# williamyang1991/VToonify

Hardware: AMD Instinct MI355X
Metric: frames/sec at 1024x1024 VToonify-D inference (higher is better)
Workload: dtype bf16

## Files before the change

include/vtoonify_amd.h:

```cpp
#ifndef VTOONIFY_AMD_H
#define VTOONIFY_AMD_H

#include <stdint.h>

#ifdef __cplusplus
extern "C" {
#endif

#define VT_ABI_VERSION 5

enum { VT_F32 = 0, VT_BF16 = 1, VT_F16 = 2,
       VT_F32X3 = 3,
       VT_F64 = 4 };
enum { VT_OK = 0, VT_ERR_ARG = 1, VT_ERR_UNSUPPORTED = 2, VT_ERR_LAUNCH = 3 };

enum { VT_ACT_NONE = 0, VT_ACT_LRELU = 1, VT_ACT_RELU_TANH = 2, VT_ACT_SIGMOID = 3, VT_ACT_TANH = 4  };
enum { VT_OUT_NHWC = 0, VT_OUT_NCHW = 1 };

typedef void* vt_stream;

int vt_abi_version(void);
const char* vt_last_error(void);
const char* vt_build_target(void);

// ... 161 lines not shown

int vt_nchw_to_nhwc(void* out, int ld_out, const void* in, int n, int c, int hw,
                    int in_dtype, int out_dtype, vt_stream stream);
int vt_nhwc_to_nchw(void* out, const void* in, int ld_in, int n, int c, int hw,
                    int in_dtype, int out_dtype, vt_stream stream);

int vt_mfma_selftest(float* c, const void* a, const void* b, int dtype, vt_stream stream);

#ifdef __cplusplus
}
#endif

#include "vtoonify_amd_prepass.h"
#include "vtoonify_amd_frames.h"
#include "vtoonify_amd_fusion.h"
#endif
```

vtoonify_amd/_lib.py:

```python
from __future__ import annotations

import ctypes as C
import os

HERE = os.path.dirname(os.path.abspath(__file__))
DEFAULT_LIB = os.path.join(HERE, "lib", "libvtoonify_amd.so")

ABI_VERSION = 5
VT_F32, VT_BF16, VT_F16 = 0, 1, 2
VT_F64 = 4
VT_F32X3 = 3
ACT_NONE, ACT_LRELU, ACT_RELU_TANH, ACT_SIGMOID, ACT_TANH = 0, 1, 2, 3, 4
OUT_NHWC, OUT_NCHW = 0, 1


class VtError(RuntimeError):
    pass


class ConvDesc(C.Structure):
    _fields_ = [
        ("src0", C.c_void_p), ("src1", C.c_void_p),
        ("c0", C.c_int32), ("c1", C.c_int32), ("ld0", C.c_int32), ("ld1", C.c_int32),
        ("n", C.c_int32), ("h", C.c_int32), ("w", C.c_int32),
# ... 116 lines not shown
}
PREPASS_SYMBOLS = tuple(_PREPASS_SIGS)

_FRAMES_SIGS = {
    "vt_frame_scale_crop": (C.c_int, [C.c_void_p, C.c_void_p] + [C.c_int] * 6 + [C.c_void_p, C.c_void_p, C.c_int, C.c_int,
                                                                               C.c_void_p]),
}
FRAMES_SYMBOLS = tuple(_FRAMES_SIGS)

_FUSION_SIGS = {
    "vt_conv2d_gate": (C.c_int, [C.POINTER(ConvDesc), C.c_void_p, C.c_int32, C.c_void_p]),
    "vt_conv2d_hdr": (C.c_int, [C.POINTER(ConvDesc), C.c_void_p, C.c_int32, C.c_int32, C.c_void_p]),
}
FUSION_SYMBOLS = tuple(_FUSION_SIGS)

_lib = None
_lib_path = None


def _bind(path: str):
    import torch
    lib = C.CDLL(path)
    for name, (res, args) in {**_SIGS, **_PREPASS_SIGS, **_FRAMES_SIGS, **_FUSION_SIGS}.items():
        fn = getattr(lib, name)
        fn.restype = res
        fn.argtypes = args
    if lib.vt_abi_version() != ABI_VERSION:
        raise VtError(f"{path}: ABI version {lib.vt_abi_version()} != {ABI_VERSION}")
    return lib


def use_library(path: str):
    global _lib, _lib_path
    _lib = _bind(path)
    _lib_path = path
    return _lib


# ... 35 lines not shown
```

vtoonify_amd/csrc/conv_igemm.hip:

```cpp
#include <stdlib.h>
#include <type_traits>
#include <utility>

#include "vt_common.hpp"

namespace {

#ifdef VT_EMU
typedef emu_f32x4 f32x4;
#else
typedef float f32x4 __attribute__((ext_vector_type(4)));
typedef __bf16 bf16x8_t __attribute__((ext_vector_type(8)));
typedef _Float16 f16x8_t __attribute__((ext_vector_type(8)));
#endif

static inline int slab_ld(int cout_total) { return (cout_total + 31) / 32 * 32; }
constexpr int64_t VT_TICKET_BYTES = 16384;

struct ConvArgs {
    const void* src0;
    const void* src1;
    const void* wgt;
    const float* bias;
    const float* slope_vec;
// ... 1337 lines not shown
        vt_lds_barrier();
        if (a_age < 99) ++a_age;
        bbuf = (bbuf + 1 == NSTB) ? 0 : bbuf + 1;
        nbbuf = (nbbuf + 1 == NSTB) ? 0 : nbbuf + 1;
        if (++tap == 9) {
            tap = 0;
            ++chunk;
            if (ABUF == 2) abuf ^= 1;
            a_age = 99;
        }
    }
    __syncthreads();
    conv_epilogue<T, BM, BN, WM, WN>(p, acc, smem, PatchRows<TW>{img, y0, x0, p.Ho, p.Wo}, n0, split, tile_n * p.tiles_m + tile_m);
}

template <typename T>
__global__ void __launch_bounds__(256, 2)
conv3x3_c32_kernel(const ConvArgs p, const GldsArgs g) {
    static_assert(is_h16<T>::value, "16-bit operands only (64-byte pixel rows)");
    constexpr int TH = 16, TW = 16, BM = 256, BN = 32, WM = 4, WN = 1;
    constexpr int TM = 4, TN = 2;
    constexpr int PH = TH + 2, PW = TW + 2, PROWS = PH * PW;
    constexpr int PA = ((PROWS + 15) / 16 + 3) / 4;
    constexpr int A_BYTES = PA * 4 * 1024;
    constexpr int NBUF = 3;
    __shared__ __attribute__((aligned(1024))) unsigned char smem[NBUF * A_BYTES];

    const int tid = threadIdx.x;
    const int lane = tid & 63;
    const int wave = vt_uniform(tid >> 6) & 3;
    const int wm = wave;
    const int q = lane >> 4, l15 = lane & 15;
    auto swz = [](int pr) -> int { return ((pr >> 2) & 1) << 1; };

// ... 36 lines not shown
        for (int i = 0; i < 4; ++i) bvr[b][i] = 0.0f;
    u128 rwf = u128{0u, 0u, 0u, 0u};
    if (rgbf) {
        const bool okw = (l15 & 3) < 3;
        const u128 wv = ld128((const T*)p.rgb_w + (okw ? (l15 & 3) * 32 + q * 8 : 0));
        rwf.x = okw ? wv.x : 0u, rwf.y = okw ? wv.y : 0u, rwf.z = okw ? wv.z : 0u, rwf.w = okw ? wv.w : 0u;
    }
    if (p.bias) {
#pragma unroll
        for (int b = 0; b < TN; ++b)
#pragma unroll
            for (int i = 0; i < 4; ++i) bvr[b][i] = p.bias[cg + frag_channel<true>(b, q) + i];
    }
    float rb0 = 0.0f, rb1 = 0.0f, rb2 = 0.0f;
    if (rgbf && p.rgb_bias) rb0 = p.rgb_bias[0], rb1 = p.rgb_bias[1], rb2 = p.rgb_bias[2];

    int tile = blockIdx.x;
    if (tile >= ntiles) return;
    issue(tile, 0);
    if (tile + (int)gridDim.x < ntiles) issue(tile + (int)gridDim.x, 1);
    int buf = 0;
    for (; tile < ntiles; tile += gridDim.x) {
        const int next2 = tile + 2 * (int)gridDim.x;
        if (next2 < ntiles) {
            issue(next2, buf == 0 ? 2 : buf - 1);
            vt_glds_wait_n<2 * PA>();
        } else if (tile + (int)gridDim.x < ntiles) {
            vt_glds_wait_n<PA>();
        } else {
            vt_glds_wait_n<0>();
// ... 1 lines not shown
        vt_lds_barrier();
        const int img = tile / (tiles_x * tiles_y);
        const int trem = tile - img * (tiles_x * tiles_y);
        const int y0 = (trem / tiles_x) * TH, x0 = (trem % tiles_x) * TW;
        const PatchRows<TW> rowmap{img, y0, x0, p.Ho, p.Wo};
        const int HoWo = p.Ho * p.Wo;
        static_assert(TM == 4, "one tile row per lane group");
        float rsd[3] = {0.0f, 0.0f, 0.0f};
        const int m_rgb = rowmap(wm * (TM * 16) + q * 16 + l15);
        int64_t o_rgb = 0;
        {
            const int mm = m_rgb < 0 ? 0 : m_rgb;
            const int im = mm / HoWo;
            o_rgb = (int64_t)im * 3 * HoWo + (mm - im * HoWo);
        }
        if (rgbf && p.rgb_resid) {
#pragma unroll
            for (int j = 0; j < 3; ++j) rsd[j] = p.rgb_resid[o_rgb + (int64_t)j * HoWo];
        }
        f32x4 acc[TM][TN];
#pragma unroll
        for (int a = 0; a < TM; ++a)
#pragma unroll
            for (int b = 0; b < TN; ++b) acc[a][b] = f32x4{0.f, 0.f, 0.f, 0.f};
        const unsigned char* sa = smem + buf * A_BYTES;
#pragma unroll
        for (int t = 0; t < 9; ++t) {
            const int ky = t / 3, kx = t - ky * 3;
            u128 fa[TM];
#pragma unroll
            for (int a = 0; a < TM; ++a) {
// ... 21 lines not shown
                        if (p.act == VT_ACT_LRELU) v = (v > 0.0f) ? v : v * p.slope;
                        f[4 * b + i] = v * ga;
                    }
                }
                const u128 fpk = pack16<T>(f);
                if (rgbf) {
                    const bool mine = (l15 >> 2) == a;
                    u128 wa;
                    wa.x = mine ? rwf.x : 0u, wa.y = mine ? rwf.y : 0u, wa.z = mine ? rwf.z : 0u, wa.w = mine ? rwf.w : 0u;
                    Mma<T>::run(racc, wa, fpk);
                }
                if (m >= 0 && !p.rgb_only) st128((T*)p.out + (int64_t)m * p.ld_out + cg + q * 8, fpk);
            }
            if (rgbf) {
                const float rr[3] = {racc[0], racc[1], racc[2]};
                if (m_rgb >= 0) {
                    p.rgb_out[o_rgb] = rr[0] + rb0 + rsd[0];
                    p.rgb_out[o_rgb + HoWo] = rr[1] + rb1 + rsd[1];
                    p.rgb_out[o_rgb + 2 * (int64_t)HoWo] = rr[2] + rb2 + rsd[2];
                }
            }
        }
        vt_lds_barrier();
        buf = buf + 1 == NBUF ? 0 : buf + 1;
    }
}

template <int... I, typename F>
__device__ __forceinline__ void vt_static_for_impl(std::integer_sequence<int, I...>, F&& f) {
    (f(std::integral_constant<int, I>{}), ...);
// ... 712 lines not shown
    if (args.phase != 2) {
        if (args.splitk == 1 && conv_lean<T>(args)) {
            auto k = conv_patchc_kernel<T, TH, BN, WM, WN, 1, DIL>;
            VT_LAUNCH(k, dim3((unsigned)blocks), dim3(WM * WN * 64), stream, args, g);
        } else {
            auto k = conv_patchc_kernel<T, TH, BN, WM, WN, 0, DIL>;
            VT_LAUNCH(k, dim3((unsigned)blocks), dim3(WM * WN * 64), stream, args, g);
        }
    }
    int rc = vt_check_launch("vt_conv2d(patch, chunk barriers)");
    if (rc != VT_OK || args.splitk == 1 || args.tickets || args.phase == 1) return rc;
    return launch_reduce<T>(args, stream);
}

template <typename T, int TH, int BN>
int launch_patchw(const ConvArgs& a, const GldsArgs& g, vt_stream stream) {
    ConvArgs args = a;
    args.slab_perm = ((BN / 16) % 2 == 0) ? 1 : 0;
    args.tiles_n = 1;
    args.tiles_m = a.N * vt_cdiv(a.Ho, TH) * vt_cdiv(a.Wo, 16);
    args.kps = 1;
    args.splitk = 1;
    split_mode(args);
    int wgs = patchw_wgs();
    if (wgs > args.tiles_m) wgs = args.tiles_m;
    if (wgs >= 8) wgs &= ~7;
    auto k = conv_patchw_kernel<T, TH, BN>;
    VT_LAUNCH(k, dim3((unsigned)wgs), dim3(512), stream, args, g);
    return vt_check_launch("vt_conv2d(patch, weights resident)");
}

template <typename T>
int launch_c32(const ConvArgs& a, const GldsArgs& g, vt_stream stream) {
    ConvArgs args = a;
    args.slab_perm = 0;
    args.splitk = 1;
    args.tiles_n = 1;
    args.tiles_m = a.N * vt_cdiv(a.Ho, 16) * vt_cdiv(a.Wo, 16);
    const int groups = a.cout / 32;
    const int per_group = 512 / groups > 0 ? 512 / groups : 1;
    int blocks = args.tiles_m < per_group ? args.tiles_m : per_group;
    if (const char* e = getenv("VT_C32_BLOCKS")) {
        const int v = atoi(e);
        if (v > 0 && v < blocks) blocks = v;
    }
    auto k = conv3x3_c32_kernel<T>;
    VT_LAUNCH(k, dim3((unsigned)blocks, (unsigned)groups), dim3(256), stream, args, g);
    return vt_check_launch("vt_conv2d(c32)");
}

template <typename T>
int dispatch(const ConvArgs& a0, int hint, int64_t ws_floats, vt_stream stream) {
    ConvArgs a = a0;
    a.force_generic = hint >= 1000000000 || !axes_equal(a);
    const TilePlan t = choose_plan<T>(a, hint % 1000000000, ws_floats);
    a.splitk = t.splitk;
    a.ldp = slab_ld(a.coutT);
    if (a.rgb_w && (t.bn < a.coutT || t.splitk > 1)) {
        vt_set_error("vt_conv2d: fused ToRGB needs all %d output channels in one tile (plan %dx%d, split %d)",
                     a.coutT, t.bm, t.bn, t.splitk);
        return VT_ERR_UNSUPPORTED;
    }
    if (a.in_absdiff && t.kind != 6) {
        vt_set_error("vt_conv2d: in_absdiff needs the thin-output kernel (plan kind %d)", t.kind);
        return VT_ERR_UNSUPPORTED;
    }
    if (a.rgb_only && t.kind != 3) {
        vt_set_error("vt_conv2d: rgb_only needs the persistent 32 -> 32 kernel (plan kind %d)", t.kind);
        return VT_ERR_UNSUPPORTED;
    }
    if (t.kind == 5) {
        const int chunks = a.cin / (8 * (16 / (int)sizeof(T)));
// ... 54 lines not shown
    }
    if (t.kind == 4) {
        FullkArgs fg;
        if (!fullk_eligible<T>(a, a.wstream, fg)) {
            vt_set_error("vt_conv2d: whole-K kernel requested for an ineligible convolution");
            return VT_ERR_UNSUPPORTED;
        }
        return launch_fullk<T>(a, fg, stream);
    }
    if (t.kind == 3) {
        GldsArgs g;
        if (!c32_eligible<T>(a, g)) {
            vt_set_error("vt_conv2d: c32 kernel requested for an ineligible convolution");
            return VT_ERR_UNSUPPORTED;
        }
        if constexpr (is_h16<T>::value) return launch_c32<T>(a, g, stream);
    }
    if (t.kind == 1 && a.transposed) {
        GldsArgs g;
        if (!up_eligible<T>(a, g)) {
            vt_set_error("vt_conv2d: transposed patch plan requested for an ineligible convolution");
            return VT_ERR_UNSUPPORTED;
        }
        return launch_patchp<T, 16, 64, 4, 2, 8, 1>(a, g, stream);
    }
    if (t.kind == 1) {
        GldsArgs g;
        if (!patch_eligible<T>(a, g)) {
            vt_set_error("vt_conv2d: patch kernel requested for an ineligible convolution");
            return VT_ERR_UNSUPPORTED;
        }
// ... 2 lines not shown
#define VT_PATCH(TH_, BN_, WM_, WN_, DIL_, NSTB_, ABUF_, COND_) \
    if (t.bm == TH_ * 16 && t.bn == BN_ && a.dil == DIL_ && (COND_))  \
        return launch_patch<T, TH_, BN_, WM_, WN_, DIL_, NSTB_, ABUF_>(a, g, stream);
        {
            const char* e = getenv("VT_PATCH_PIPE");
            const bool pipe = !(e && e[0] == '0') && !a.x3;
            if constexpr (is_h16<T>::value) {
                const bool lean = a.coutT == 64 && a.phases == 1 && a.out_layout == VT_OUT_NHWC && !a.out_f32 && a.vec_store &&
                                  a.ld_out % 8 == 0 && !a.resid && !a.slope_vec && !a.alpha_dev && !a.post_relu && !a.stats_part &&
                                  (a.act == VT_ACT_NONE || a.act == VT_ACT_LRELU) &&
                                  (int64_t)a.N * a.Ho * a.Wo * a.ld_out * 2 < (((int64_t)1 << 31) - 4096) &&
                                  (int64_t)a.N * a.Ho * a.Wo * 12 < (((int64_t)1 << 31) - 4096);
                if (pipe && !(e && e[0] == '1') && a.dil == 1 && t.bm == 256 && t.bn == 64 && units == 1 && lean && !a.src1 &&
                    a.splitk <= 1 &&
                    (int64_t)(batch_exact() ? 1 : a.N) * vt_cdiv(a.Ho, 16) * vt_cdiv(a.Wo, 16) >= 2 * patchw_wgs())
                    return launch_patchw<T, 16, 64>(a, g, stream);
            }
            if constexpr (is_h16<T>::value) {
                if (pipe && !(e && e[0] == '1') && a.dil == 1 && t.bm == 256 && (t.bn == 128 || t.bn == 64) && a.splitk <= 1 &&
                    conv_lean<T>(a) && vt_cdiv(a.coutT, t.bn) * t.bn * 8 <= PQ_TAB_BYTES &&
                    (int64_t)a.N * vt_cdiv(a.Ho, 16) * vt_cdiv(a.Wo, 16) * vt_cdiv(a.coutT, t.bn) > patchw_wgs()) {
                    if (t.bn == 128) return launch_patchq<T, 16, 128, 4, 2, 4>(a, g, stream);
                    return launch_patchq<T, 16, 64, 4, 2, 4>(a, g, stream);
                }
            }
            if (pipe && a.dil == 1 && t.bm == 256 && t.bn == 128) return launch_patchp<T, 16, 128, 4, 2>(a, g, stream);
            if (pipe && a.dil == 1 && t.bm == 256 && t.bn == 64) return launch_patchp<T, 16, 64, 4, 2, 4>(a, g, stream);
            if constexpr (is_h16<T>::value) {
                if (pipe && !(e && e[0] == '1') && a.dil == 1 && t.bm == 256 && t.bn == 32) return launch_patchc<T>(a, g, stream);
                if (pipe && !(e && e[0] == '1') && a.dil == 2 && t.bm == 256 && t.bn == 32 && !a.stats_part)
                    return launch_patchc<T, 2>(a, g, stream);
// ... 204 lines not shown
        vt_set_error("vt_conv2d_hdr: needs a 3x3, pad 1 conv of one source with cout <= 3");
        return VT_ERR_UNSUPPORTED;
    }
    if (hdr_c < 0 || hdr_pad <= 0 || hdr_c > hdr_pad || hdr_pad % kstep != 0) {
        vt_set_error("vt_conv2d_hdr: needs 0 <= hdr_c <= hdr_pad, hdr_pad a positive multiple of the K step (%d channels)", kstep);
        return VT_ERR_UNSUPPORTED;
    }
    a.hdr = hdr_planes;
    a.hdr_c = hdr_c;
    a.hdr_pad = hdr_pad;
    a.cin = d->c0 + hdr_pad;
    a.K = a.taps * a.cin;
    return fusion_form_run(d, a, "vt_conv2d_hdr", stream);
}

extern "C" int vt_conv2d_tile(const vt_conv_desc* d) {
    ConvArgs a;
    if (fill_args(d, a) != VT_OK) return -1;
    a.force_generic = d->tile_hint >= 1000000000 || !axes_equal(a);
    const int64_t wsf = (d->splitk_ws && d->splitk_ws_bytes > VT_TICKET_BYTES) ? (d->splitk_ws_bytes - VT_TICKET_BYTES) / 4 : 0;
    const TilePlan t = plan_of(d, a, wsf);
    int kind = t.kind;
    if (kind == 0) {
        GldsArgs g;
        const bool glds = d->dtype == VT_F16    ? glds_eligible<f16_t>(a, g)
                          : d->dtype == VT_BF16 ? glds_eligible<bf16_t>(a, g)
                                                : glds_eligible<float>(a, g);
        kind = glds ? 2 : 0;
    }
    int bm = t.bm, bn = t.bn;
// ... 95 lines not shown
```

vtoonify_amd/csrc/conv_patch_resident.hpp:

```cpp
#pragma once

template <typename T, int TH, int BN>
__global__ void __launch_bounds__(512)
conv_patchw_kernel(const ConvArgs p, const GldsArgs g) {
    constexpr int TW = 16;
    constexpr int GW = 4;
    constexpr int BM = TH * TW;
    constexpr int ESZ = (int)sizeof(T);
    constexpr int TM = BM / GW / 16, TN = BN / 16;
    constexpr bool PERM = (TN % 2 == 0);
    constexpr int PH = TH + 2, PW = TW + 2, PROWS = PH * PW;
    constexpr int NPIECE = (PROWS + 7) / 8;
    constexpr int PA = (NPIECE + GW - 1) / GW;
    constexpr int WPIECE = (BN + 7) / 8;
    constexpr int LB = (WPIECE + 7) / 8;
    constexpr int A_BYTES = NPIECE * 1024, W_TAP = WPIECE * 1024, W_BYTES = 9 * W_TAP;
    constexpr int A_OFF = W_BYTES, TAB_OFF = W_BYTES + 2 * A_BYTES;
    static_assert(sizeof(T) == 2, "bf16 (the lean epilogue packs 8 channels into a 16-byte store)");
    static_assert(BM % (GW * 16) == 0 && BN % 16 == 0, "wave tiling");
    static_assert(TM * GW == TH, "one 16-pixel tile row per MFMA row block");
    static_assert(TAB_OFF + 4 * BN * 4 <= 160 * 1024, "LDS budget");
    static_assert(TM == 4 && TN == 4, "the epilogue below: 4 tile rows per wave (one per lane group), 2 x 32 channels");
    static_assert(9 * LB + PA < 64, "vmcnt is 6 bits");

// ... 58 lines not shown
            if (piece < NPIECE) vt_glds16(r0, smem + aoff + piece * 1024, vo, 0u);
        }
    };
    if (ng > 0) issue_patch(tile_of(0));
    const bool rgbf = p.rgb_w != nullptr;
    if (tid < BN) {
        float* tab = reinterpret_cast<float*>(smem + TAB_OFF);
        tab[tid] = p.bias ? p.bias[tid] : 0.0f;
#pragma unroll
        for (int j = 0; j < 3; ++j) tab[(1 + j) * BN + tid] = rgbf ? to_f32(((const T*)p.rgb_w)[j * p.coutT + tid]) : 0.0f;
    }
    float rb[3] = {0.0f, 0.0f, 0.0f};
    if (rgbf && p.rgb_bias) rb[0] = p.rgb_bias[0], rb[1] = p.rgb_bias[1], rb[2] = p.rgb_bias[2];
    const int HoWo = p.Ho * p.Wo;
    const BufRaw rout = vt_make_raw(p.out, (uint32_t)((int64_t)p.M * p.ld_out * ESZ));
    const BufRaw rskip = vt_make_raw(p.rgb_resid, (uint32_t)((int64_t)p.N * 3 * HoWo * 4));
    const BufRaw rimg = vt_make_raw(p.rgb_out, (uint32_t)((int64_t)p.N * 3 * HoWo * 4));

    const int q = lane >> 4, l15 = lane & 15, l7 = lane & 7;
    uint32_t aswz[8][2];
#pragma unroll
    for (int cm = 0; cm < 8; ++cm)
#pragma unroll
        for (int sub = 0; sub < 2; ++sub)
            aswz[cm][sub] = (uint32_t)(aoff + (wm * TM * PW + l15) * 128 + (((sub * 4 + q) ^ ((wm * TM * PW + l15 + cm) & 7)) << 4));
    uint32_t bfix[2];
#pragma unroll
    for (int sub = 0; sub < 2; ++sub) bfix[sub] = (uint32_t)(l15 * 128 + (((sub * 4 + q) ^ l7) << 4));

    u128 fa[2][TM], fb[2][TN];
    auto read_frags = [&](auto tapc, auto subc, u128 (&xa)[TM], u128 (&xb)[TN]) {
        constexpr int TAP = decltype(tapc)::value, SUB = decltype(subc)::value;
        constexpr int ky = TAP / 3, kx = TAP % 3;
        auto ra = [&](int a) {
// ... 37 lines not shown
        });
        vt_sched_fence();
        vt_lds_barrier();
        if (j + 1 < ng) issue_patch(tile_of(j + 1));
        {
            const int tm = tile_of(j);
            const int im = tm / per_img, tr = tm - im * per_img;
            const PatchRows<TW> rowmap{im, (tr / tiles_x) * TH, (tr % tiles_x) * TW, p.Ho, p.Wo};
            const int m_rgb = rowmap(wm * (TM * 16) + q * 16 + l15);
            uint32_t o_rgb = GLDS_OOB;
            if (m_rgb >= 0) {
                const int ii = m_rgb / HoWo;
                o_rgb = (uint32_t)(ii * 3 * HoWo + (m_rgb - ii * HoWo)) * 4u;
            }
            u128 rsd[3];
            if (rgbf) {
#pragma unroll
                for (int jc = 0; jc < 3; ++jc) vt_bload_hidden<1>(rsd[jc], rskip, m_rgb >= 0 ? o_rgb + (uint32_t)(jc * HoWo) * 4u : GLDS_OOB);
            }
            const float ga = p.gain_alpha;
            const float* tab = reinterpret_cast<const float*>(smem + TAB_OFF);
            f32x4 racc = f32x4{0.f, 0.f, 0.f, 0.f};
            static_assert(TM <= 4 && sizeof(T) == 2, "ToRGB accumulator rows");
#pragma unroll
            for (int hp = 0; hp < 2; ++hp) {
                const int c0 = hp * 32 + q * 8;
                float bv[8];
                unpack16<float>(ld128(tab + c0), bv), unpack16<float>(ld128(tab + c0 + 4), bv + 4);
                u128 wfrag = u128{0u, 0u, 0u, 0u};
                if (rgbf) {
                    const int pl = (l15 & 3) < 3 ? (l15 & 3) : 0;
// ... 17 lines not shown
                    if (rgbf) {
                        const bool mine = (l15 >> 2) == a;
                        u128 wa;
                        wa.x = mine ? wfrag.x : 0u, wa.y = mine ? wfrag.y : 0u, wa.z = mine ? wfrag.z : 0u, wa.w = mine ? wfrag.w : 0u;
                        Mma<T>::run(racc, wa, fpk);
                    }
                    vt_bstore_hidden<4>(rout, m >= 0 ? (uint32_t)(m * p.ld_out + c0) * (uint32_t)ESZ : GLDS_OOB, fpk);
                }
            }
            if (rgbf) {
                const float rr[3] = {racc[0], racc[1], racc[2]};
                vt_vmcnt_fence<2 * TM>();
#pragma unroll
                for (int jc = 0; jc < 3; ++jc) {
                    u128 o;
                    o.x = vt_f2u((rr[jc] + rb[jc]) + vt_u2f(vt_settled(rsd[jc]).x)), o.y = o.z = o.w = 0u;
                    vt_bstore_hidden<1>(rimg, m_rgb >= 0 ? o_rgb + (uint32_t)(jc * HoWo) * 4u : GLDS_OOB, o);
                }
            } else {
                vt_vmcnt_fence<2 * TM>();
            }
        }
        vt_lds_barrier();
    }
    for (int k = grp + 2 * ng; k < nmine + 1; ++k) vt_lds_barrier();
}
```

vtoonify_amd/csrc/vt_common.hpp:

```cpp
#pragma once

#ifndef VT_EMU
#include <hip/hip_runtime.h>
#endif
#include <stdint.h>
#include <stdio.h>
#include <string.h>

#include "../../include/vtoonify_amd.h"

void vt_set_error(const char* fmt, ...);
int vt_check_launch(const char* what);

#define VT_REQUIRE(cond, ...)            \
    do {                                 \
        if (!(cond)) {                   \
            vt_set_error(__VA_ARGS__);   \
            return VT_ERR_ARG;           \
        }                                \
    } while (0)

#ifdef VT_EMU
#define VT_LAUNCH(kern, grid, block, stream, ...) \
    emu::launch((grid), (block), [=]() { kern(__VA_ARGS__); })
// ... 442 lines not shown
    else asm volatile("s_nop 4\n\t" OP_ " %0, %1, %2, 0 offen" ::"v"(X_), "v"(voff), "s"(r.v) : "memory");
    if constexpr (DW == 4) {
        const vt_u32x4 x = __builtin_bit_cast(vt_u32x4, v);
        VT_BST("buffer_store_dwordx4", x)
    } else if constexpr (DW == 2) {
        typedef uint32_t vt_u32x2 __attribute__((ext_vector_type(2)));
        const vt_u32x2 x = {v.x, v.y};
        VT_BST("buffer_store_dwordx2", x)
    } else {
        const uint32_t x = v.x;
        VT_BST("buffer_store_dword", x)
    }
#undef VT_BST
}
#endif

__device__ __forceinline__ float wave_sum(float v) {
#pragma unroll
    for (int off = 32; off > 0; off >>= 1) v += __shfl_xor(v, off, 64);
    return v;
}

static inline int vt_cdiv(int64_t a, int64_t b) { return (int)((a + b - 1) / b); }
__device__ __forceinline__ int vt_cdiv_dev(int a, int b) { return (a + b - 1) / b; }

#ifdef VT_EMU
static inline void vt_wave_sync() {
    const int dummy = 0;
    (void)emu::exchange(&dummy, (int)sizeof(dummy));
}
// ... 17 lines not shown
```

vtoonify_amd/engine.py:

```python
from __future__ import annotations

import ctypes as C
import math
import os
from typing import Dict, List, Optional, Tuple

import torch

from . import _lib
from . import kernels as K
from ._lib import ACT_LRELU, ACT_NONE, ACT_RELU_TANH, OUT_NCHW, OUT_NHWC

SQRT2 = math.sqrt(2.0)
N_LATENT = 18
_DIL = {1: 4, 2: 4, 3: 2, 4: 2, 5: 1, 6: 1}
SKIP_HDR = 64


def _pad8(c: int) -> int:
    return (c + 7) // 8 * 8


class _Plan:
    def __init__(self):
# ... 2 lines not shown
        self.enc_ops: List[Tuple] = []
        self.gen_ops: List[Tuple] = []
        self.keep: list = []
        self.masks: List[torch.Tensor] = []
        self.graphs: dict = {}
        self.convs: list = []


class VToonifyEngine:
    supports_borrow = True

    def __init__(self, state_dict: Dict[str, torch.Tensor], backbone: str = "dualstylegan",
                 in_size: int = 256, dtype: torch.dtype = torch.bfloat16,
                 device: Optional[torch.device] = None, cache_styles: bool = False,
                 tile_hints: Optional[Dict[str, int]] = None, style_gate: bool = False, x3: bool = False,
                 fuse_rgb128: bool = True, fused_gate=True):
        assert backbone in ("dualstylegan", "toonify")
        assert dtype in (torch.bfloat16, torch.float16, torch.float32)
        self.backbone = backbone
        self.dual = backbone == "dualstylegan"
        self.in_size = in_size
        self.dtype = dtype
        self.dt = K.dt_code(dtype)
        self.x3 = bool(x3) and dtype == torch.float32
        self.dt_conv = K.VT_F32X3 if self.x3 else self.dt
        self.h16 = dtype in (torch.bfloat16, torch.float16)
        self.precision = ({torch.bfloat16: "bf16", torch.float16: "fp16"}[dtype] if self.h16 else
                          ("fp32x3" if self.x3 else "fp32_exact"))
        self.esz = 2 if self.h16 else 4
        any_t = next(iter(state_dict.values()))
        self.device = torch.device(device) if device is not None else any_t.device
        if self.device.type == "cuda" and self.device.index is None:
            self.device = torch.device("cuda", torch.cuda.current_device())
        self.lib = _lib.lib()
        if self.device.type != "cuda" and not _lib.is_emulation():
            raise _lib.VtError("VToonifyEngine needs a GPU device (no CPU path)")
        self.cache_styles = cache_styles
        self.fuse_rgb128 = bool(fuse_rgb128)
        self.fused_gate = fused_gate if fused_gate == "all" else bool(fused_gate)
        self.style_gate = bool(style_gate)
        self.graph_first = os.environ.get("VT_GRAPH_FIRST", "1") != "0"
        self.use_upblur = True
        self.tile_hints: Dict[str, int] = dict(tile_hints or {})
        if not self.tile_hints and os.environ.get("VT_TILE_HINTS"):
            import json
            with open(os.environ["VT_TILE_HINTS"]) as f:
                self.tile_hints = {k: int(v) for k, v in json.load(f).items()}
        self.sd = {k: v.detach().to(self.device, torch.float32).contiguous() for k, v in state_dict.items()}
        self.g = "generator.generator." if self.dual else "generator."
        self.n_down = 0
        while f"encoder.{self.n_down}.0.weight" in self.sd:
            self.n_down += 1
        self.n_fuse = sum(1 for lvl in range(5) if 2 ** (5 + lvl) <= in_size)
        import collections
# ... 103 lines not shown
            info["join"] = True
        if entry is not None:
            info["form"] = entry[2]
            info["bytes"] += entry[3]
        plan.convs.append((d, info, ops, len(ops)))
        ops.append((self.lib.vt_conv2d, (C.byref(d),), info) if entry is None else (entry[0], (C.byref(d),) + tuple(entry[1]), info))

    def _conv_kind(self, **kw) -> int:
        wt = kw.get("weight")
        if isinstance(wt, torch.Tensor) and wt.data_ptr() in self._wstream:
            kw["weight_stream"] = self._wstream[wt.data_ptr()]
        d = self._apply_hint(K.make_conv_desc(dtype=self.dt_conv, **kw))
        d.splitk_ws, d.splitk_ws_bytes = 1 << 20, 1 << 40
        tile = self.lib.vt_conv2d_tile(C.byref(d))
        return tile // 100000000 if tile >= 0 else -1

    def _op_linear(self, ops, y, ld_y, x, ld_x, W, b, rows, w_scale=1.0, b_scale=1.0, act=ACT_NONE,
                   slope=0.2, gain=1.0):
        out_dim, in_dim = W.shape
        ops.append((self.lib.vt_linear,
                    (C.c_void_p(K._ptr(y)), ld_y, C.c_void_p(K._ptr(x)), ld_x, C.c_void_p(W.data_ptr()),
                     C.c_void_p(b.data_ptr() if b is not None else 0), rows, in_dim, out_dim,
                     float(w_scale), float(b_scale), act, float(slope), float(gain)), "linear"))

    @staticmethod
    def _info(what):
        if isinstance(what, dict):
            return what
        return {"name": what, "kernel": what, "flops": 0, "bytes": 0}

# ... 317 lines not shown
                sk2 = self._buf(plan, f"fskip{lvl}", (B, 3, h, w), f32)
                skip_kw = dict(n=B, h=h, w=w, out_h=h, out_w=w, weight=self.w[f"fusion_skip.{lvl}"], cout=3, kh=3, kw=3, pad=1,
                               bias=sd[f"fusion_skip.{lvl}.bias"], out=sk2, ld_out=0, out_layout=OUT_NCHW,
                               out_dtype=K.VT_F32, branch=1)
                if fused:
                    self._op_conv(ops, plan, src0=fem, c0=co, ld0=co, **skip_kw,
                                  entry=(lib.vt_conv2d_hdr, (C.c_void_p(skip.data_ptr()), 3, SKIP_HDR), "+hdr", B * hw * 12))
                else:
                    self._op_conv(ops, plan, src0=fem, c0=co + hdr, ld0=co + hdr, **skip_kw)
                out, skip = fo, sk2
            n1, n2, n3 = f"convs.{6 + 2 * lvl}", f"convs.{7 + 2 * lvl}", f"to_rgbs.{3 + lvl}"
            c1o = self.modw[n1].shape[0]
            up = self._buf(plan, f"up{lvl}", (B, 2 * h, 2 * w, c1o))
            o2 = self._buf(plan, f"gout{lvl}", (B, 2 * h, 2 * w, c1o))
            rgb = self._buf(plan, f"rgb{lvl}", (B, 3, 2 * h, 2 * w), f32)
            ops.append((lib.vt_upfirdn2d,
                        (C.c_void_p(rgb.data_ptr()), C.c_void_p(skip.data_ptr()), C.c_void_p(self.fir_rgb.data_ptr()),
                         B * 3, h, w, 4, 4, 2, 2, 1, 1, 2, 1, 2, 1, K.VT_F32),
                        {"name": "upfirdn2d", "kernel": "upfirdn2d_tile<f32,up2>", "flops": 0, "branch": 1,
                         "bytes": B * 3 * hw * 5 * 4}))
            groups = [(0, B)] if ns == 1 else [(b, 1) for b in range(B)]
            for b0, nb in groups:
                sidx = 0 if ns == 1 else b0
                wm1 = plan.modw[n1][sidx]
                wm2 = plan.modw[n2][sidx]
                wm3 = plan.modw[n3][sidx]
                ref_macs = nb * hw * co * c1o * 9 + nb * 4 * hw * c1o * 16
                if self.use_upblur:
                    self._op_conv(ops, plan, ref_macs=ref_macs, src0=out.data_ptr() + b0 * hw * co * self.esz, c0=co,
                                  ld0=co, n=nb, h=h, w=w, out_h=2 * h, out_w=2 * w, weight=wm1, cout=c1o, kh=3, kw=3,
                                  up_fir=self.fir_up, bias=sd[f"{g}{n1}.activate.bias"], act=ACT_LRELU, gain=SQRT2,
                                  out=up.data_ptr() + b0 * 4 * hw * c1o * self.esz, ld_out=c1o)
                else:
                    self._op_conv(ops, plan, ref_macs=ref_macs, src0=out.data_ptr() + b0 * hw * co * self.esz, c0=co,
                                  ld0=co, n=nb, h=h, w=w, out_h=h, out_w=w, weight=wm1, cout=c1o, kh=3, kw=3, pad=1,
                                  phases=4, bias=sd[f"{g}{n1}.activate.bias"], act=ACT_LRELU, gain=SQRT2,
                                  out=up.data_ptr() + b0 * 4 * hw * c1o * self.esz, ld_out=c1o)
                same_kw = dict(src0=up.data_ptr() + b0 * 4 * hw * c1o * self.esz, c0=c1o, ld0=c1o, n=nb,
                               h=2 * h, w=2 * w, out_h=2 * h, out_w=2 * w, weight=wm2, cout=c1o, kh=3, kw=3, pad=1,
                               bias=sd[f"{g}{n2}.activate.bias"], act=ACT_LRELU, gain=SQRT2,
                               out=o2.data_ptr() + b0 * 4 * hw * c1o * self.esz, ld_out=c1o)
                rgb_ptr = rgb.data_ptr() + b0 * 3 * 4 * hw * 4
                rgb_kw = dict(rgb_weight=wm3, rgb_bias=self.w[f"{n3}.bias"], rgb_resid=rgb_ptr, rgb_out=rgb_ptr)
                probe = self._apply_hint(K.make_conv_desc(dtype=self.dt_conv, **same_kw, **rgb_kw))
                probe.splitk_ws, probe.splitk_ws_bytes = 1 << 20, 1 << 40
                tile = self.lib.vt_conv2d_tile(C.byref(probe))
                fuse_rgb = tile >= 0 and tile % 1000 >= c1o and (tile // 1000000) % 100 <= 1
                if fuse_rgb and not self.fuse_rgb128 and self.h16 and tile // 100000000 == 1 and tile % 1000 == 128:
                    fuse_rgb = False
                rgb_only = fuse_rgb and lvl == 4 and tile // 100000000 == 3
                self._op_conv(ops, plan, join=fuse_rgb, **same_kw, **(rgb_kw if fuse_rgb else {}),
                              **({"rgb_only": 1} if rgb_only else {}))
                if not fuse_rgb:
                    self._op_conv(ops, plan, join=True, src0=o2.data_ptr() + b0 * 4 * hw * c1o * self.esz, c0=c1o, ld0=c1o, n=nb,
                                  h=2 * h, w=2 * w, out_h=2 * h, out_w=2 * w, weight=wm3, cout=3, kh=1, kw=1,
                                  bias=self.w[f"{n3}.bias"], beta=1.0, resid=rgb_ptr, out=rgb_ptr, ld_out=0,
                                  out_layout=OUT_NCHW, out_dtype=K.VT_F32)
            out, co, skip, h, w = o2, c1o, rgb, 2 * h, 2 * w
        plan.image = skip
        self._finalize_convs(plan)
        return plan

    def _finalize_convs(self, plan: _Plan):
        need = {}
        for d, info, _, _ in plan.convs:
# ... 227 lines not shown
```

vtoonify_amd/kernels.py:

```python
from __future__ import annotations

import ctypes as C

import torch

from . import _lib
from ._lib import ACT_LRELU, ACT_NONE, ACT_RELU_TANH, OUT_NCHW, OUT_NHWC, VT_BF16, VT_F16, VT_F32, VT_F32X3, VT_F64, ConvDesc

_DT = {torch.float32: VT_F32, torch.bfloat16: VT_BF16, torch.float16: VT_F16}


def dt_code(dtype: torch.dtype) -> int:
    try:
        return _DT[dtype]
    except KeyError:
        raise _lib.VtError(f"unsupported dtype {dtype}") from None


def op_dt_code(dtype: torch.dtype) -> int:
    return VT_F64 if dtype == torch.float64 else dt_code(dtype)


def _dev_ok(*tensors):
    for t in tensors:
# ... 121 lines not shown
    _lib.check(_lib.lib().vt_conv2d(C.byref(d), _stream(t)), "vt_conv2d")


def conv2d_gate(fem, ld_fem, *, stream_of=None, **kw):
    d = make_conv_desc(**kw)
    t = stream_of if stream_of is not None else (kw["out"] if isinstance(kw["out"], torch.Tensor) else kw["src0"])
    _lib.check(_lib.lib().vt_conv2d_gate(C.byref(d), _ptr(fem), int(ld_fem), _stream(t)), "vt_conv2d_gate")


def conv2d_hdr(hdr_planes, hdr_c, hdr_pad, *, stream_of=None, **kw):
    d = make_conv_desc(**kw)
    t = stream_of if stream_of is not None else (kw["out"] if isinstance(kw["out"], torch.Tensor) else kw["src0"])
    _lib.check(_lib.lib().vt_conv2d_hdr(C.byref(d), _ptr(hdr_planes), int(hdr_c), int(hdr_pad), _stream(t)), "vt_conv2d_hdr")


def pack_conv_weight(w: torch.Tensor, cin_dst=None, chan_map=None, scale=1.0, src_transposed=False,
                     out_dtype=torch.float32):
    _dev_ok(w, chan_map)
    if src_transposed:
        cin_src, cout, kh, kw = w.shape
    else:
        cout, cin_src, kh, kw = w.shape
    cin_dst = cin_dst or (cin_src + 7) // 8 * 8
    out = torch.empty((cout, kh * kw, cin_dst), dtype=out_dtype, device=w.device)
    _lib.check(_lib.lib().vt_pack_conv_weight(_p(out), _p(w), cout, cin_src, kh, kw, cin_dst, _p(chan_map),
                                             float(scale), int(src_transposed), dt_code(out_dtype),
                                             _stream(w)), "vt_pack_conv_weight")
    return out


# ... 123 lines not shown
```

Measured before the change: 1671.

## Fold ToRGB skip upfirdn2d upsample into the fused conv epilogue

Removes the separate upfirdn2d launch that upsamples the lower-resolution RGB skip image. Instead, the fused ToRGB epilogue in the c32 and weights-resident patch conv kernels reads the 2x2 lo-res window directly and applies the 4x4 FIR taps, chosen per lane by output parity. This saves one kernel launch plus the full-resolution skip write and read-back, in exchange for extra gathers and FMAs in the conv epilogue and a new variadic template path.

```diff
diff --git a/include/vtoonify_amd.h b/include/vtoonify_amd.h
--- a/include/vtoonify_amd.h
+++ b/include/vtoonify_amd.h
@@ -199,4 +199,5 @@
 #include "vtoonify_amd_prepass.h"
 #include "vtoonify_amd_frames.h"
 #include "vtoonify_amd_fusion.h"
+#include "vtoonify_amd_rgbup.h"
 #endif
diff --git a/include/vtoonify_amd_rgbup.h b/include/vtoonify_amd_rgbup.h
--- /dev/null
+++ b/include/vtoonify_amd_rgbup.h
@@ -0,0 +1,14 @@
+#ifndef VTOONIFY_AMD_RGBUP_H
+#define VTOONIFY_AMD_RGBUP_H
+#include "vtoonify_amd.h"
+
+#ifdef __cplusplus
+extern "C" {
+#endif
+
+int vt_conv2d_rgbup(const vt_conv_desc* conv, const float* lo_planes, const float* fir, vt_stream stream);
+
+#ifdef __cplusplus
+}
+#endif
+#endif
diff --git a/vtoonify_amd/_lib.py b/vtoonify_amd/_lib.py
--- a/vtoonify_amd/_lib.py
+++ b/vtoonify_amd/_lib.py
@@ -154,6 +154,11 @@
 }
 FUSION_SYMBOLS = tuple(_FUSION_SIGS)
 
+_RGBUP_SIGS = {
+    "vt_conv2d_rgbup": (C.c_int, [C.POINTER(ConvDesc), C.c_void_p, C.c_void_p, C.c_void_p]),
+}
+RGBUP_SYMBOLS = tuple(_RGBUP_SIGS)
+
 _lib = None
 _lib_path = None
 
@@ -161,7 +166,7 @@
 def _bind(path: str):
     import torch
     lib = C.CDLL(path)
-    for name, (res, args) in {**_SIGS, **_PREPASS_SIGS, **_FRAMES_SIGS, **_FUSION_SIGS}.items():
+    for name, (res, args) in {**_SIGS, **_PREPASS_SIGS, **_FRAMES_SIGS, **_FUSION_SIGS, **_RGBUP_SIGS}.items():
         fn = getattr(lib, name)
         fn.restype = res
         fn.argtypes = args
diff --git a/vtoonify_amd/csrc/conv_igemm.hip b/vtoonify_amd/csrc/conv_igemm.hip
--- a/vtoonify_amd/csrc/conv_igemm.hip
+++ b/vtoonify_amd/csrc/conv_igemm.hip
@@ -1375,10 +1375,48 @@
     conv_epilogue<T, BM, BN, WM, WN>(p, acc, smem, PatchRows<TW>{img, y0, x0, p.Ho, p.Wo}, n0, split, tile_n * p.tiles_m + tile_m);
 }
 
-template <typename T>
+struct SkipUpArgs {
+    const float* lo;
+    const float* fir;
+    int h, w;
+};
+__device__ __forceinline__ void skipup_taps(const float* fir, int py, int px, float (&uw)[4]) {
+#pragma unroll
+    for (int jy = 0; jy < 2; ++jy)
+#pragma unroll
+        for (int jx = 0; jx < 2; ++jx) uw[2 * jy + jx] = fir[(3 - py - 2 * jy) * 4 + (3 - px - 2 * jx)];
+}
+__device__ __forceinline__ void skipup_window(int Y, int X, int h, int w, int (&off)[4], bool (&ok)[4]) {
+    const int r0 = ((Y + 1) >> 1) - 1, c0 = ((X + 1) >> 1) - 1;
+#pragma unroll
+    for (int jy = 0; jy < 2; ++jy)
+#pragma unroll
+        for (int jx = 0; jx < 2; ++jx) {
+            const int r = r0 + jy, c = c0 + jx;
+            ok[2 * jy + jx] = (unsigned)r < (unsigned)h && (unsigned)c < (unsigned)w;
+            const int rc = r < 0 ? 0 : (r >= h ? h - 1 : r), cc = c < 0 ? 0 : (c >= w ? w - 1 : c);
+            off[2 * jy + jx] = rc * w + cc;
+        }
+}
+template <typename... UP>
+__device__ __forceinline__ SkipUpArgs skipup_of(const UP&... up) {
+    static_assert(sizeof...(UP) <= 1, "no argument or one SkipUpArgs");
+    if constexpr (sizeof...(UP) == 1) return (up, ...);
+    else return SkipUpArgs{nullptr, nullptr, 0, 0};
+}
+__device__ __forceinline__ float skipup_value(const float (&v)[4], const bool (&ok)[4], const float (&uw)[4]) {
+    float a = 0.0f;
+#pragma unroll
+    for (int t = 0; t < 4; ++t) a = fmaf(ok[t] ? v[t] : 0.0f, uw[t], a);
+    return a;
+}
+
+template <typename T, typename... UP>
 __global__ void __launch_bounds__(256, 2)
-conv3x3_c32_kernel(const ConvArgs p, const GldsArgs g) {
+conv3x3_c32_kernel(const ConvArgs p, const GldsArgs g, const UP... up) {
     static_assert(is_h16<T>::value, "16-bit operands only (64-byte pixel rows)");
+    constexpr bool UPF = sizeof...(UP) == 1;
+    const SkipUpArgs u = skipup_of(up...);
     constexpr int TH = 16, TW = 16, BM = 256, BN = 32, WM = 4, WN = 1;
     constexpr int TM = 4, TN = 2;
     constexpr int PH = TH + 2, PW = TW + 2, PROWS = PH * PW;
@@ -1445,6 +1483,9 @@
     }
     float rb0 = 0.0f, rb1 = 0.0f, rb2 = 0.0f;
     if (rgbf && p.rgb_bias) rb0 = p.rgb_bias[0], rb1 = p.rgb_bias[1], rb2 = p.rgb_bias[2];
+    static_assert(TH % 2 == 0 && TW % 2 == 0 && TM % 2 == 0, "the output parity of a lane's pixel does not depend on the tile");
+    float uw[4] = {0.0f, 0.0f, 0.0f, 0.0f};
+    if constexpr (UPF) skipup_taps(u.fir, q & 1, l15 & 1, uw);
 
     int tile = blockIdx.x;
     if (tile >= ntiles) return;
@@ -1476,7 +1517,17 @@
             const int im = mm / HoWo;
             o_rgb = (int64_t)im * 3 * HoWo + (mm - im * HoWo);
         }
-        if (rgbf && p.rgb_resid) {
+        float ulo[3][4];
+        bool uok[4];
+        if constexpr (UPF) {
+            int uoff[4];
+            skipup_window(y0 + wm * TM + q, x0 + l15, u.h, u.w, uoff, uok);
+            const float* lo = u.lo + (int64_t)img * 3 * u.h * u.w;
+#pragma unroll
+            for (int j = 0; j < 3; ++j)
+#pragma unroll
+                for (int t = 0; t < 4; ++t) ulo[j][t] = lo[j * (u.h * u.w) + uoff[t]];
+        } else if (rgbf && p.rgb_resid) {
 #pragma unroll
             for (int j = 0; j < 3; ++j) rsd[j] = p.rgb_resid[o_rgb + (int64_t)j * HoWo];
         }
@@ -1528,6 +1579,10 @@
             }
             if (rgbf) {
                 const float rr[3] = {racc[0], racc[1], racc[2]};
+                if constexpr (UPF) {
+#pragma unroll
+                    for (int j = 0; j < 3; ++j) rsd[j] = skipup_value(ulo[j], uok, uw);
+                }
                 if (m_rgb >= 0) {
                     p.rgb_out[o_rgb] = rr[0] + rb0 + rsd[0];
                     p.rgb_out[o_rgb + HoWo] = rr[1] + rb1 + rsd[1];
@@ -2270,7 +2325,7 @@
 }
 
 template <typename T, int TH, int BN>
-int launch_patchw(const ConvArgs& a, const GldsArgs& g, vt_stream stream) {
+int launch_patchw(const ConvArgs& a, const GldsArgs& g, vt_stream stream, const SkipUpArgs* su = nullptr) {
     ConvArgs args = a;
     args.slab_perm = ((BN / 16) % 2 == 0) ? 1 : 0;
     args.tiles_n = 1;
@@ -2281,13 +2336,18 @@
     int wgs = patchw_wgs();
     if (wgs > args.tiles_m) wgs = args.tiles_m;
     if (wgs >= 8) wgs &= ~7;
-    auto k = conv_patchw_kernel<T, TH, BN>;
+    if (su) {
+        void (*k)(const ConvArgs, const GldsArgs, const SkipUpArgs) = conv_patchw_kernel<T, TH, BN, SkipUpArgs>;
+        VT_LAUNCH(k, dim3((unsigned)wgs), dim3(512), stream, args, g, *su);
+        return vt_check_launch("vt_conv2d_rgbup(patch, weights resident)");
+    }
+    void (*k)(const ConvArgs, const GldsArgs) = conv_patchw_kernel<T, TH, BN>;
     VT_LAUNCH(k, dim3((unsigned)wgs), dim3(512), stream, args, g);
     return vt_check_launch("vt_conv2d(patch, weights resident)");
 }
 
 template <typename T>
-int launch_c32(const ConvArgs& a, const GldsArgs& g, vt_stream stream) {
+int launch_c32(const ConvArgs& a, const GldsArgs& g, vt_stream stream, const SkipUpArgs* su = nullptr) {
     ConvArgs args = a;
     args.slab_perm = 0;
     args.splitk = 1;
@@ -2300,18 +2360,29 @@
         const int v = atoi(e);
         if (v > 0 && v < blocks) blocks = v;
     }
-    auto k = conv3x3_c32_kernel<T>;
+    if (su) {
+        void (*k)(const ConvArgs, const GldsArgs, const SkipUpArgs) = conv3x3_c32_kernel<T, SkipUpArgs>;
+        VT_LAUNCH(k, dim3((unsigned)blocks, (unsigned)groups), dim3(256), stream, args, g, *su);
+        return vt_check_launch("vt_conv2d_rgbup(c32)");
+    }
+    void (*k)(const ConvArgs, const GldsArgs) = conv3x3_c32_kernel<T>;
     VT_LAUNCH(k, dim3((unsigned)blocks, (unsigned)groups), dim3(256), stream, args, g);
     return vt_check_launch("vt_conv2d(c32)");
 }
 
 template <typename T>
-int dispatch(const ConvArgs& a0, int hint, int64_t ws_floats, vt_stream stream) {
+int dispatch(const ConvArgs& a0, int hint, int64_t ws_floats, vt_stream stream, const SkipUpArgs* su = nullptr) {
     ConvArgs a = a0;
     a.force_generic = hint >= 1000000000 || !axes_equal(a);
     const TilePlan t = choose_plan<T>(a, hint % 1000000000, ws_floats);
     a.splitk = t.splitk;
     a.ldp = slab_ld(a.coutT);
+    if (su && t.kind != 3 && t.kind != 1) {
+        vt_set_error("vt_conv2d_rgbup: the descriptor runs on neither the persistent 32 -> 32 kernel nor the weights-resident "
+                     "patch form (plan kind %d)", t.kind);
+        return VT_ERR_UNSUPPORTED;
+    }
+
     if (a.rgb_w && (t.bn < a.coutT || t.splitk > 1)) {
         vt_set_error("vt_conv2d: fused ToRGB needs all %d output channels in one tile (plan %dx%d, split %d)",
                      a.coutT, t.bm, t.bn, t.splitk);
@@ -2396,7 +2467,7 @@
             vt_set_error("vt_conv2d: c32 kernel requested for an ineligible convolution");
             return VT_ERR_UNSUPPORTED;
         }
-        if constexpr (is_h16<T>::value) return launch_c32<T>(a, g, stream);
+        if constexpr (is_h16<T>::value) return launch_c32<T>(a, g, stream, su);
     }
     if (t.kind == 1 && a.transposed) {
         GldsArgs g;
@@ -2429,7 +2500,11 @@
                 if (pipe && !(e && e[0] == '1') && a.dil == 1 && t.bm == 256 && t.bn == 64 && units == 1 && lean && !a.src1 &&
                     a.splitk <= 1 &&
                     (int64_t)(batch_exact() ? 1 : a.N) * vt_cdiv(a.Ho, 16) * vt_cdiv(a.Wo, 16) >= 2 * patchw_wgs())
-                    return launch_patchw<T, 16, 64>(a, g, stream);
+                    return launch_patchw<T, 16, 64>(a, g, stream, su);
+            }
+            if (su) {
+                vt_set_error("vt_conv2d_rgbup: the descriptor does not run on the weights-resident patch form (tile %dx%d)", t.bm, t.bn);
+                return VT_ERR_UNSUPPORTED;
             }
             if constexpr (is_h16<T>::value) {
                 if (pipe && !(e && e[0] == '1') && a.dil == 1 && t.bm == 256 && (t.bn == 128 || t.bn == 64) && a.splitk <= 1 &&
@@ -2664,6 +2739,27 @@
     return fusion_form_run(d, a, "vt_conv2d_hdr", stream);
 }
 
+extern "C" int vt_conv2d_rgbup(const vt_conv_desc* d, const float* lo_planes, const float* fir, vt_stream stream) {
+    ConvArgs a;
+    const int rc = fill_args(d, a);
+    if (rc != VT_OK) return rc;
+    VT_REQUIRE(lo_planes && fir, "vt_conv2d_rgbup: null planes or FIR");
+    if (!a.rgb_w || a.stats_part) {
+        vt_set_error("vt_conv2d_rgbup: needs a conv with the fused ToRGB (rgb_weight) and without stats_part");
+        return VT_ERR_UNSUPPORTED;
+    }
+    if (d->out_h % 2 != 0 || d->out_w % 2 != 0) {
+        vt_set_error("vt_conv2d_rgbup: the output (%d x %d) is not twice a lo-res image", d->out_h, d->out_w);
+        return VT_ERR_UNSUPPORTED;
+    }
+    a.rgb_resid = nullptr;
+    const SkipUpArgs su{lo_planes, fir, d->out_h / 2, d->out_w / 2};
+    const int64_t wsf = (d->splitk_ws && d->splitk_ws_bytes > VT_TICKET_BYTES) ? (d->splitk_ws_bytes - VT_TICKET_BYTES) / 4 : 0;
+    return d->dtype == VT_F16    ? dispatch<f16_t>(a, d->tile_hint, wsf, stream, &su)
+           : d->dtype == VT_BF16 ? dispatch<bf16_t>(a, d->tile_hint, wsf, stream, &su)
+                                 : dispatch<float>(a, d->tile_hint, wsf, stream, &su);
+}
+
 extern "C" int vt_conv2d_tile(const vt_conv_desc* d) {
     ConvArgs a;
     if (fill_args(d, a) != VT_OK) return -1;
diff --git a/vtoonify_amd/csrc/conv_patch_resident.hpp b/vtoonify_amd/csrc/conv_patch_resident.hpp
--- a/vtoonify_amd/csrc/conv_patch_resident.hpp
+++ b/vtoonify_amd/csrc/conv_patch_resident.hpp
@@ -1,8 +1,10 @@
 #pragma once
 
-template <typename T, int TH, int BN>
+template <typename T, int TH, int BN, typename... UP>
 __global__ void __launch_bounds__(512)
-conv_patchw_kernel(const ConvArgs p, const GldsArgs g) {
+conv_patchw_kernel(const ConvArgs p, const GldsArgs g, const UP... up) {
+    constexpr bool UPF = sizeof...(UP) == 1;
+    const SkipUpArgs u = skipup_of(up...);
     constexpr int TW = 16;
     constexpr int GW = 4;
     constexpr int BM = TH * TW;
@@ -96,10 +98,14 @@
     if (rgbf && p.rgb_bias) rb[0] = p.rgb_bias[0], rb[1] = p.rgb_bias[1], rb[2] = p.rgb_bias[2];
     const int HoWo = p.Ho * p.Wo;
     const BufRaw rout = vt_make_raw(p.out, (uint32_t)((int64_t)p.M * p.ld_out * ESZ));
-    const BufRaw rskip = vt_make_raw(p.rgb_resid, (uint32_t)((int64_t)p.N * 3 * HoWo * 4));
+    const BufRaw rskip = UPF ? vt_make_raw(u.lo, (uint32_t)((int64_t)p.N * 3 * u.h * u.w * 4))
+                             : vt_make_raw(p.rgb_resid, (uint32_t)((int64_t)p.N * 3 * HoWo * 4));
     const BufRaw rimg = vt_make_raw(p.rgb_out, (uint32_t)((int64_t)p.N * 3 * HoWo * 4));
 
     const int q = lane >> 4, l15 = lane & 15, l7 = lane & 7;
+    static_assert(TH % 2 == 0 && TW % 2 == 0 && TM % 2 == 0, "the output parity of a lane's pixel does not depend on the tile");
+    float uw[4] = {0.0f, 0.0f, 0.0f, 0.0f};
+    if constexpr (UPF) skipup_taps(u.fir, q & 1, l15 & 1, uw);
     uint32_t aswz[8][2];
 #pragma unroll
     for (int cm = 0; cm < 8; ++cm)
@@ -167,7 +173,21 @@
                 o_rgb = (uint32_t)(ii * 3 * HoWo + (m_rgb - ii * HoWo)) * 4u;
             }
             u128 rsd[3];
-            if (rgbf) {
+            uint32_t ulo[3][4];
+            if constexpr (UPF) {
+                static_assert(PA + 12 + 2 * TM + 3 < 64, "vmcnt is 6 bits");
+                if (rgbf) {
+                    int uoff[4];
+                    bool uok[4];
+                    skipup_window(rowmap.y0 + wm * TM + q, rowmap.x0 + l15, u.h, u.w, uoff, uok);
+                    const int hw_lo = u.h * u.w;
+#pragma unroll
+                    for (int jc = 0; jc < 3; ++jc)
+#pragma unroll
+                        for (int t = 0; t < 4; ++t)
+                            vt_bload_hidden_u32(ulo[jc][t], rskip, uok[t] ? (uint32_t)((im * 3 + jc) * hw_lo + uoff[t]) * 4u : GLDS_OOB);
+                }
+            } else if (rgbf) {
 #pragma unroll
                 for (int jc = 0; jc < 3; ++jc) vt_bload_hidden<1>(rsd[jc], rskip, m_rgb >= 0 ? o_rgb + (uint32_t)(jc * HoWo) * 4u : GLDS_OOB);
             }
@@ -215,7 +235,14 @@
 #pragma unroll
                 for (int jc = 0; jc < 3; ++jc) {
                     u128 o;
-                    o.x = vt_f2u((rr[jc] + rb[jc]) + vt_u2f(vt_settled(rsd[jc]).x)), o.y = o.z = o.w = 0u;
+                    if constexpr (UPF) {
+                        float skv = 0.0f;
+#pragma unroll
+                        for (int t = 0; t < 4; ++t) skv = fmaf(vt_u2f(vt_settled_u32(ulo[jc][t])), uw[t], skv);
+                        o.x = vt_f2u((rr[jc] + rb[jc]) + skv), o.y = o.z = o.w = 0u;
+                    } else {
+                        o.x = vt_f2u((rr[jc] + rb[jc]) + vt_u2f(vt_settled(rsd[jc]).x)), o.y = o.z = o.w = 0u;
+                    }
                     vt_bstore_hidden<1>(rimg, m_rgb >= 0 ? o_rgb + (uint32_t)(jc * HoWo) * 4u : GLDS_OOB, o);
                 }
             } else {
diff --git a/vtoonify_amd/csrc/vt_common.hpp b/vtoonify_amd/csrc/vt_common.hpp
--- a/vtoonify_amd/csrc/vt_common.hpp
+++ b/vtoonify_amd/csrc/vt_common.hpp
@@ -480,6 +480,21 @@
 #undef VT_BST
 }
 #endif
+#ifdef VT_EMU
+static inline void vt_bload_hidden_u32(uint32_t& v, const BufRaw& r, uint32_t voff) {
+    v = 0u;
+    if ((uint64_t)voff + 4 <= r.nrec) memcpy(&v, r.base + voff, 4);
+}
+static inline uint32_t vt_settled_u32(uint32_t v) { return v; }
+#else
+__device__ __forceinline__ void vt_bload_hidden_u32(uint32_t& v, const BufRaw& r, uint32_t voff) {
+    asm volatile("s_nop 4\n\tbuffer_load_dword %0, %1, %2, 0 offen" : "=&v"(v) : "v"(voff), "s"(r.v));
+}
+__device__ __forceinline__ uint32_t vt_settled_u32(uint32_t v) {
+    asm volatile("" : "+v"(v));
+    return v;
+}
+#endif
 
 __device__ __forceinline__ float wave_sum(float v) {
 #pragma unroll
diff --git a/vtoonify_amd/engine.py b/vtoonify_amd/engine.py
--- a/vtoonify_amd/engine.py
+++ b/vtoonify_amd/engine.py
@@ -40,7 +40,7 @@
                  in_size: int = 256, dtype: torch.dtype = torch.bfloat16,
                  device: Optional[torch.device] = None, cache_styles: bool = False,
                  tile_hints: Optional[Dict[str, int]] = None, style_gate: bool = False, x3: bool = False,
-                 fuse_rgb128: bool = True, fused_gate=True):
+                 fuse_rgb128: bool = True, fused_gate=True, fold_rgb_up: bool = True):
         assert backbone in ("dualstylegan", "toonify")
         assert dtype in (torch.bfloat16, torch.float16, torch.float32)
         self.backbone = backbone
@@ -64,6 +64,7 @@
         self.cache_styles = cache_styles
         self.fuse_rgb128 = bool(fuse_rgb128)
         self.fused_gate = fused_gate if fused_gate == "all" else bool(fused_gate)
+        self.fold_rgb_up = bool(fold_rgb_up)
         self.style_gate = bool(style_gate)
         self.graph_first = os.environ.get("VT_GRAPH_FIRST", "1") != "0"
         self.use_upblur = True
@@ -197,6 +198,21 @@
         d.splitk_ws, d.splitk_ws_bytes = 1 << 20, 1 << 40
         tile = self.lib.vt_conv2d_tile(C.byref(d))
         return tile // 100000000 if tile >= 0 else -1
+
+    def _rgbup_resident(self, tile: int, n: int, ho: int, wo: int, cout: int) -> bool:
+        if os.environ.get("VT_PATCH_PIPE", "")[:1] in ("0", "1") or os.environ.get("VT_BATCH_EXACT", "")[:1] == "1":
+            return False
+        kind, sk, bm, bn = tile // 100000000, (tile // 1000000) % 100, (tile // 1000) % 1000, tile % 1000
+        return (kind == 1 and sk <= 1 and bm == 256 and bn == 64 and cout == 64 and
+                n * ((ho + 15) // 16) * ((wo + 15) // 16) >= 2 * self._patchw_wgs())
+
+    def _patchw_wgs(self) -> int:
+        e = os.environ.get("VT_PATCHW_WGS", "")
+        if e.isdigit() and int(e) > 0:
+            return int(e)
+        if self.device.type == "cuda":
+            return torch.cuda.get_device_properties(self.device).multi_processor_count
+        return 256
 
     def _op_linear(self, ops, y, ld_y, x, ld_x, W, b, rows, w_scale=1.0, b_scale=1.0, act=ACT_NONE,
                    slope=0.2, gain=1.0):
@@ -544,16 +560,37 @@
             up = self._buf(plan, f"up{lvl}", (B, 2 * h, 2 * w, c1o))
             o2 = self._buf(plan, f"gout{lvl}", (B, 2 * h, 2 * w, c1o))
             rgb = self._buf(plan, f"rgb{lvl}", (B, 3, 2 * h, 2 * w), f32)
-            ops.append((lib.vt_upfirdn2d,
-                        (C.c_void_p(rgb.data_ptr()), C.c_void_p(skip.data_ptr()), C.c_void_p(self.fir_rgb.data_ptr()),
-                         B * 3, h, w, 4, 4, 2, 2, 1, 1, 2, 1, 2, 1, K.VT_F32),
-                        {"name": "upfirdn2d", "kernel": "upfirdn2d_tile<f32,up2>", "flops": 0, "branch": 1,
-                         "bytes": B * 3 * hw * 5 * 4}))
             groups = [(0, B)] if ns == 1 else [(b, 1) for b in range(B)]
+
+            def same_conv(b0, nb):
+                sidx = 0 if ns == 1 else b0
+                same_kw = dict(src0=up.data_ptr() + b0 * 4 * hw * c1o * self.esz, c0=c1o, ld0=c1o, n=nb,
+                               h=2 * h, w=2 * w, out_h=2 * h, out_w=2 * w, weight=plan.modw[n2][sidx], cout=c1o, kh=3, kw=3, pad=1,
+                               bias=sd[f"{g}{n2}.activate.bias"], act=ACT_LRELU, gain=SQRT2,
+                               out=o2.data_ptr() + b0 * 4 * hw * c1o * self.esz, ld_out=c1o)
+                rgb_ptr = rgb.data_ptr() + b0 * 3 * 4 * hw * 4
+                rgb_kw = dict(rgb_weight=plan.modw[n3][sidx], rgb_bias=self.w[f"{n3}.bias"], rgb_resid=rgb_ptr, rgb_out=rgb_ptr)
+                probe = self._apply_hint(K.make_conv_desc(dtype=self.dt_conv, **same_kw, **rgb_kw))
+                probe.splitk_ws, probe.splitk_ws_bytes = 1 << 20, 1 << 40
+                tile = self.lib.vt_conv2d_tile(C.byref(probe))
+                fuse_rgb = tile >= 0 and tile % 1000 >= c1o and (tile // 1000000) % 100 <= 1
+                if fuse_rgb and not self.fuse_rgb128 and self.h16 and tile // 100000000 == 1 and tile % 1000 == 128:
+                    fuse_rgb = False
+                rgb_only = fuse_rgb and lvl == 4 and tile // 100000000 == 3
+                return same_kw, rgb_kw, tile, fuse_rgb, rgb_only
+
+            _, _, tile0, fuse0, _ = same_conv(*groups[0])
+            fold_up = (self.fold_rgb_up and fuse0 and self.h16 and
+                       (tile0 // 100000000 == 3 or self._rgbup_resident(tile0, groups[0][1], 2 * h, 2 * w, c1o)))
+            if not fold_up:
+                ops.append((lib.vt_upfirdn2d,
+                            (C.c_void_p(rgb.data_ptr()), C.c_void_p(skip.data_ptr()), C.c_void_p(self.fir_rgb.data_ptr()),
+                             B * 3, h, w, 4, 4, 2, 2, 1, 1, 2, 1, 2, 1, K.VT_F32),
+                            {"name": "upfirdn2d", "kernel": "upfirdn2d_tile<f32,up2>", "flops": 0, "branch": 1,
+                             "bytes": B * 3 * hw * 5 * 4}))
             for b0, nb in groups:
                 sidx = 0 if ns == 1 else b0
                 wm1 = plan.modw[n1][sidx]
-                wm2 = plan.modw[n2][sidx]
                 wm3 = plan.modw[n3][sidx]
                 ref_macs = nb * hw * co * c1o * 9 + nb * 4 * hw * c1o * 16
                 if self.use_upblur:
@@ -566,19 +603,14 @@
                                   ld0=co, n=nb, h=h, w=w, out_h=h, out_w=w, weight=wm1, cout=c1o, kh=3, kw=3, pad=1,
                                   phases=4, bias=sd[f"{g}{n1}.activate.bias"], act=ACT_LRELU, gain=SQRT2,
                                   out=up.data_ptr() + b0 * 4 * hw * c1o * self.esz, ld_out=c1o)
-                same_kw = dict(src0=up.data_ptr() + b0 * 4 * hw * c1o * self.esz, c0=c1o, ld0=c1o, n=nb,
-                               h=2 * h, w=2 * w, out_h=2 * h, out_w=2 * w, weight=wm2, cout=c1o, kh=3, kw=3, pad=1,
-                               bias=sd[f"{g}{n2}.activate.bias"], act=ACT_LRELU, gain=SQRT2,
-                               out=o2.data_ptr() + b0 * 4 * hw * c1o * self.esz, ld_out=c1o)
-                rgb_ptr = rgb.data_ptr() + b0 * 3 * 4 * hw * 4
-                rgb_kw = dict(rgb_weight=wm3, rgb_bias=self.w[f"{n3}.bias"], rgb_resid=rgb_ptr, rgb_out=rgb_ptr)
-                probe = self._apply_hint(K.make_conv_desc(dtype=self.dt_conv, **same_kw, **rgb_kw))
-                probe.splitk_ws, probe.splitk_ws_bytes = 1 << 20, 1 << 40
-                tile = self.lib.vt_conv2d_tile(C.byref(probe))
-                fuse_rgb = tile >= 0 and tile % 1000 >= c1o and (tile // 1000000) % 100 <= 1
-                if fuse_rgb and not self.fuse_rgb128 and self.h16 and tile // 100000000 == 1 and tile % 1000 == 128:
-                    fuse_rgb = False
-                rgb_only = fuse_rgb and lvl == 4 and tile // 100000000 == 3
+                same_kw, rgb_kw, tile, fuse_rgb, rgb_only = same_conv(b0, nb)
+                rgb_ptr = rgb_kw["rgb_out"]
+                if fold_up:
+                    lo_ptr = skip.data_ptr() + b0 * 3 * hw * 4
+                    self._op_conv(ops, plan, join=True, **same_kw, **rgb_kw, **({"rgb_only": 1} if rgb_only else {}),
+                                  entry=(lib.vt_conv2d_rgbup, (C.c_void_p(lo_ptr), C.c_void_p(self.fir_rgb.data_ptr())), ".up",
+                                         nb * 3 * hw * 4))
+                    continue
                 self._op_conv(ops, plan, join=fuse_rgb, **same_kw, **(rgb_kw if fuse_rgb else {}),
                               **({"rgb_only": 1} if rgb_only else {}))
                 if not fuse_rgb:
diff --git a/vtoonify_amd/kernels.py b/vtoonify_amd/kernels.py
--- a/vtoonify_amd/kernels.py
+++ b/vtoonify_amd/kernels.py
@@ -159,6 +159,12 @@
     _lib.check(_lib.lib().vt_conv2d_hdr(C.byref(d), _ptr(hdr_planes), int(hdr_c), int(hdr_pad), _stream(t)), "vt_conv2d_hdr")
 
 
+def conv2d_rgbup(lo_planes, fir, *, stream_of=None, **kw):
+    d = make_conv_desc(**kw)
+    t = stream_of if stream_of is not None else (kw["out"] if isinstance(kw["out"], torch.Tensor) else kw["src0"])
+    _lib.check(_lib.lib().vt_conv2d_rgbup(C.byref(d), _ptr(lo_planes), _ptr(fir), _stream(t)), "vt_conv2d_rgbup")
+
+
 def pack_conv_weight(w: torch.Tensor, cin_dst=None, chan_map=None, scale=1.0, src_transposed=False,
                      out_dtype=torch.float32):
     _dev_ok(w, chan_map)
```

Measured after the change: 1691, median of 6. +1.2%, better.
